# LiliMeng/network_interpretation_imagenet

Hardware: AMD Instinct MI355X
Metric: masked-forward-passes/sec (224x224, resnet101) (higher is better)
Workload: dtype f16x3 (split-fp16 MFMA, fp32 accumulate); stem conv in fp32 by superposition over superpixels; 1 GPU; resnet101, 512 masks/image x 128 images per GPU (BASELINE configs[2]; x1 GPUs); images_per_gpu=128, masks_per_image=512, forward_batch=2340, num_cus=256, entry=MaskedForwardEngine.score_packed, stem=table, lib_stamp=cd5194694597393f7e4ba467b20fff02ebc9e9c5ea24d07d825e02e5c1091293, lib_stamp_matches_tree=True, product_library=True, parallelism=mask-batch shard x1 + one all_gather of scores

## Files before the change

### network_interpretation_imagenet_amd/csrc/mpx_api.hip

```cpp
#include "../../include/mpx.h"
#include "mpx_kernels.h"
#include "mpx_conv3p.h"
#include "mpx_conv3pp.h"
#include "mpx_conv256.h"
#include "mpx_conv256p.h"
#include "mpx_convx.h"
#include "mpx_convw.h"
#include "mpx_btail.h"
#include "mpx_stemtab.h"
#include "mpx_dw.h"
#include "mpx_fire.h"
#include "mpx_pool3c.h"
#include "mpx_shuffle.h"
#include "mpx_mbconv.h"
#include "mpx_gconv.h"
#include "mpx_gconvw.h"
#include "mpx_cnext.h"
#include "mpx_attn.h"

#include <algorithm>
#include <cmath>
#include <cstdarg>
#include <initializer_list>
#include <new>
// ... 141 lines not shown
    int side, bf, hp, a_pitch, b_pitch, b_offset;
};

struct ClipPool {
    int hin, stride, pad, pitch;
};

struct ProfRec {
    hipEvent_t t0, t1;
    int kind;
    int conv;
    int sub;
};

}

struct mpx_engine {
    int arch = 0, max_batch = 0, device = 0;
    int num_cus = 256;
    int img = MPX_IMG, in_ch = 3, ncls = MPX_NUM_CLASSES, logit_pitch = MPX_NUM_CLASSES;
    bool small = false;
    bool vgg = false;
    bool alexnet = false;
    bool densenet = false;
    std::vector<NormLayer> norms;
    bool mobilenet = false;
    std::vector<DwLayer> dws;
    bool squeezenet = false;
    bool googlenet = false;
    std::vector<ClipPool> pools3c;
    bool shufflenet = false;
    std::vector<ShuffleOp> shuffles;
    bool efficientnet = false;
    std::vector<SeLayer> ses;
    float* se_gate = nullptr;
    int se_pitch_max = 0;
    bool convnext = false;
    std::vector<LnLayer> lnorms;
    bool regnet = false;
    bool vit = false;
    int vit_T = 0, vit_D = 0;
    std::vector<AttnLayer> attns;
    float* cls_token = nullptr;
    float* pos_emb = nullptr;
    bool tokens_loaded = false;
    size_t act_elems_buf[4] = {0, 0, 0, 0};
    int n_act_bufs = kActBufs;
    size_t act_elems_per_image = 0;
    float* k0_scratch = nullptr;
    bool bottleneck = false;
    int feat = 0;
    std::vector<ConvLayer> convs;
    std::vector<Op> ops;
    std::vector<Op> ops_bt;
    std::vector<TailBlock> tails;
    int ops_bt_x = 0;
    bool fuse_bt = true;
    std::vector<Op> ops_pt;
    std::vector<Op> ops_pt0;
    std::vector<PointTail> ptails;
    int ops_pt_x = 0, ops_pt0_x = 0;
    bool fuse_pt = true;
    char* arena = nullptr;
    size_t arena_bytes = 0;
    char* tab_arena = nullptr;
    size_t tab_arena_bytes = 0;
    half_t* in_hi = nullptr;
    half_t* in_lo = nullptr;
    half_t* act_hi[kActBufs] = {};
    half_t* act_lo[kActBufs] = {};
    half_t* pool_hi = nullptr;
    half_t* pool_lo = nullptr;
    float* logits = nullptr;
    float* seg_scratch = nullptr;
    half_t* stem_hi = nullptr;
    half_t* stem_lo = nullptr;
    float* stem_w32 = nullptr;
    float* stem_s32 = nullptr;
    float* stem_t32 = nullptr;
    int* tab_cnt = nullptr;
    int* tab_off = nullptr;
    int* tab_lab = nullptr;
    int* tab_heavy = nullptr;
    float* tab_vec = nullptr;
    unsigned* tab_bits = nullptr;
    size_t tab_sizes[4] = {0, 0, 0, 0};
    int tab_S = -1;
    bool stem_w_loaded = false;
    std::vector<uint8_t> slot_src;
    std::string err;
    bool in_forward = false;
    unsigned last_kernels = 0;
    bool fuse_ds = true;
    bool fuse_pool = true;
    bool prof_on = false;
    std::vector<ProfRec> prof_pool;
    int prof_used = 0;
    hipStream_t prof_stream = nullptr;
#ifdef MPX_DIAG
    unsigned long long* stamps = nullptr;
#endif
};

namespace {

int fail(mpx_engine* h, int code, const char* fmt, ...) {
    if (h) {
        char buf[512];
        va_list ap;
        va_start(ap, fmt);
        vsnprintf(buf, sizeof buf, fmt, ap);
        va_end(ap);
        h->err = buf;
    }
    return code;
}

#define MPX_HIP(h, call)                                                                         \
    do {                                                                                         \
        hipError_t e_ = (call);                                                                  \
        if (e_ != hipSuccess)                                                                    \
            return fail((h), (int)e_, "%s failed: %s (%s:%d)", #call, hipGetErrorString(e_),     \
                        __FILE__, __LINE__);                                                     \
    } while (0)

#define MPX_SET_DEVICE(h)                                   \
    do {                                                    \
        if (!(h)->in_forward) MPX_HIP((h), hipSetDevice((h)->device)); \
    } while (0)

size_t round_up(size_t v, size_t a) { return (v + a - 1) / a * a; }

void set_name(char* dst, const std::string& s) {
    std::snprintf(dst, 48, "%s", s.c_str());
}

int default_tile(const mpx_conv_desc& d);
bool patch_eligible(const mpx_conv_desc& d);

constexpr int kGconvTile = 16;
constexpr int kGconvwTile = 18;

int build_topology_small(mpx_engine* h);
int build_topology_vgg(mpx_engine* h);
int build_topology_alexnet(mpx_engine* h);
int build_topology_densenet(mpx_engine* h);
int build_topology_mobilenet(mpx_engine* h);
int build_topology_squeezenet(mpx_engine* h);
int build_topology_googlenet(mpx_engine* h);
int build_topology_shufflenet(mpx_engine* h);
int build_topology_efficientnet(mpx_engine* h);
int build_topology_convnext(mpx_engine* h);
int build_topology_vit(mpx_engine* h);
int build_topology_regnet(mpx_engine* h);

int build_topology(mpx_engine* h) {
    if (h->arch == MPX_ARCH_MNIST_NET || (h->arch > MPX_ARCH_CIFAR_RESNET && h->arch < MPX_ARCH_CIFAR_RESNET + 1000))
        return build_topology_small(h);
    if (h->arch > MPX_ARCH_VGG && h->arch < MPX_ARCH_VGG_BN + 100) return build_topology_vgg(h);
    if (h->arch >= MPX_ARCH_ALEXNET && h->arch < MPX_ARCH_ALEXNET + 100) return build_topology_alexnet(h);
    if (h->arch >= MPX_ARCH_DENSENET && h->arch < MPX_ARCH_DENSENET + 1000) return build_topology_densenet(h);
    if (h->arch >= MPX_ARCH_MOBILENET && h->arch < MPX_ARCH_MOBILENET + 1000) return build_topology_mobilenet(h);
    if (h->arch >= MPX_ARCH_SQUEEZENET && h->arch < MPX_ARCH_SQUEEZENET + 1000) return build_topology_squeezenet(h);
    if (h->arch >= MPX_ARCH_GOOGLENET && h->arch < MPX_ARCH_GOOGLENET + 1000) return build_topology_googlenet(h);
    if (h->arch >= MPX_ARCH_SHUFFLENET && h->arch < MPX_ARCH_SHUFFLENET + 1000) return build_topology_shufflenet(h);
    if (h->arch >= MPX_ARCH_EFFICIENTNET && h->arch < MPX_ARCH_EFFICIENTNET + 1000) return build_topology_efficientnet(h);
// ... 2448 lines not shown
    if (bias) *bias = h->lnorms[k].beta;
    if (eps) *eps = h->lnorms[k].eps;
    return 0;
}

int mpx_num_norms(const mpx_engine* h) { return h ? (int)h->norms.size() : MPX_E_ARG; }

int mpx_norm_info(const mpx_engine* h, int k, mpx_norm_desc* out) {
    if (!h || !out || k < 0 || k >= (int)h->norms.size()) return MPX_E_ARG;
    *out = h->norms[k].d;
    return 0;
}

int mpx_load_norm(mpx_engine* h, int k, const float* gamma, const float* beta, const float* mean, const float* var, float eps) {
    if (!h) return MPX_E_ARG;
    if (k < 0 || k >= (int)h->norms.size()) return fail(h, MPX_E_ARG, "load_norm: bad norm index %d (this engine has %d)", k, (int)h->norms.size());
    NormLayer& nl = h->norms[k];
    if (!gamma || !beta || !mean || !var) return fail(h, MPX_E_ARG, "load_norm: BatchNorm tensors missing for %s", nl.d.name);
    const int n = nl.d.channels;
    std::vector<float> sc(n), sh(n);
    for (int c = 0; c < n; ++c) {
        const double s = (double)gamma[c] / std::sqrt((double)var[c] + (double)eps);
        sc[c] = (float)s;
        sh[c] = (float)((double)beta[c] - (double)mean[c] * s);
    }
    MPX_SET_DEVICE(h);
    MPX_HIP(h, hipMemcpy(nl.scale, sc.data(), (size_t)n * 4, hipMemcpyHostToDevice));
    MPX_HIP(h, hipMemcpy(nl.shift, sh.data(), (size_t)n * 4, hipMemcpyHostToDevice));
    nl.loaded = true;
    return 0;
}

int mpx_norm_params(const mpx_engine* h, int k, const float** scale, const float** shift) {
    if (!h || !scale || !shift || k < 0 || k >= (int)h->norms.size()) return MPX_E_ARG;
    *scale = h->norms[k].scale;
    *shift = h->norms[k].shift;
    return 0;
}

int mpx_mask_apply_normalize(mpx_engine* h, const uint8_t* img_u8_hwc, const float* img_f32_chw, const int32_t* seg,
                             const uint8_t* onoff, int M, int S, const float mean[3], const float std[3], int slot0,
                             float* out_f32_nchw, void* stream) {
    if (!h) return MPX_E_ARG;
    if (h->small) return fail(h, MPX_E_STATE, "mask_apply_normalize: this engine runs one of the small networks; use mpx_mask_apply_minmax");
    if ((img_u8_hwc == nullptr) == (img_f32_chw == nullptr))
        return fail(h, MPX_E_ARG, "mask_apply_normalize: exactly one of img_u8_hwc / img_f32_chw must be given");
    if (!seg || !onoff || M <= 0 || S <= 0) return fail(h, MPX_E_ARG, "mask_apply_normalize: null input or empty M/S");
    if (img_u8_hwc && (!mean || !std)) return fail(h, MPX_E_ARG, "mask_apply_normalize: mean/std required for u8 input");
    if (slot0 < 0 || slot0 + M > h->max_batch) return fail(h, MPX_E_STATE, "mask_apply_normalize: slots [%d,%d) exceed max_batch %d", slot0, slot0 + M, h->max_batch);
    const size_t lds = round_up((size_t)K0_MT * S, 16);
    if (lds > 64 * 1024) return fail(h, MPX_E_ARG, "mask_apply_normalize: S=%d too large (max %d)", S, 64 * 1024 / K0_MT);
    MaskParams p;
    std::memset(&p, 0, sizeof p);
    p.img_u8 = img_u8_hwc; p.img_f32 = img_f32_chw; p.seg = seg; p.onoff = onoff;
    p.out_hi = h->in_hi; p.out_lo = h->in_lo; p.out_f32 = out_f32_nchw;
    for (int c = 0; c < 3; ++c) {
        p.mean[c] = mean ? mean[c] : 0.f;
        p.std[c] = std ? std[c] : 1.f;
    }
    p.M = M; p.S = S; p.slot0 = slot0;
    p.size = MPX_IMG; p.pad_size = MPX_IMG_PAD; p.border = 3;
    MPX_SET_DEVICE(h);
    hipStream_t st = as_stream(stream);
    ProfScope ps(h, st, 1, -1);
    dim3 grid((MPX_IMG * MPX_IMG + 255) / 256, (M + K0_MT - 1) / K0_MT);
    hipLaunchKernelGGL(mask_apply_normalize_kernel, grid, dim3(256), lds, st, p);
    MPX_HIP(h, hipGetLastError());
    std::fill(h->slot_src.begin() + slot0, h->slot_src.begin() + slot0 + M, (uint8_t)1);
    return 0;
}

int mpx_stem_table_build(mpx_engine* h, const uint8_t* img_u8_hwc, const float* img_f32_chw, const int32_t* seg, int S,
                         const float mean[3], const float std[3], void* stream) {
    if (!h) return MPX_E_ARG;
    if (h->densenet) return fail(h, MPX_E_STATE, "stem_table_build: a DenseNet engine keeps no stem table; it stages through mpx_mask_apply_normalize");
    if (!h->stem_w32) return fail(h, MPX_E_STATE, "stem_table_build: this architecture has no 7x7 stem with a max pool%s", h->vgg || h->alexnet || h->mobilenet || h->squeezenet || h->googlenet || h->shufflenet || h->efficientnet || h->convnext || h->vit || h->regnet ? " (VGG, AlexNet, MobileNetV2, SqueezeNet, GoogLeNet, ShuffleNetV2, EfficientNet-B0, ConvNeXt, ViT and RegNetX stage through mpx_mask_apply_normalize)" : "");
    if ((img_u8_hwc == nullptr) == (img_f32_chw == nullptr))
        return fail(h, MPX_E_ARG, "stem_table_build: exactly one of img_u8_hwc / img_f32_chw must be given");
    if (!seg || S <= 0 || S > 4096) return fail(h, MPX_E_ARG, "stem_table_build: null label map or S outside [1, 4096]");
    if (img_u8_hwc && (!mean || !std)) return fail(h, MPX_E_ARG, "stem_table_build: mean/std required for u8 input");
    if (!h->stem_w_loaded) return fail(h, MPX_E_STATE, "stem_table_build: layer 0 (%s) has no weights", h->convs[0].d.name);
    MPX_SET_DEVICE(h);
    if (!h->tab_arena) {
        const size_t total = 3 * h->tab_sizes[0] + h->tab_sizes[1] + h->tab_sizes[2] + h->tab_sizes[3];
        MPX_HIP(h, hipMalloc((void**)&h->tab_arena, total));
        h->tab_arena_bytes = total;
        char* cur = h->tab_arena;
        auto take = [&](size_t n) { char* r = cur; cur += n; return r; };
        h->tab_cnt = (int*)take(h->tab_sizes[0]);
        h->tab_off = (int*)take(h->tab_sizes[0]);
        h->tab_heavy = (int*)take(h->tab_sizes[0]);
        h->tab_lab = (int*)take(h->tab_sizes[1]);
        h->tab_vec = (float*)take(h->tab_sizes[2]);
        h->tab_bits = (unsigned*)take(h->tab_sizes[3]);
    }
    StemTabParams p;
    std::memset(&p, 0, sizeof p);
    p.img_u8 = img_u8_hwc; p.img_f32 = img_f32_chw; p.seg = seg; p.S = S;
    for (int c = 0; c < 3; ++c) {
        p.mean[c] = mean ? mean[c] : 0.f;
        p.std[c] = std ? std[c] : 1.f;
    }
    p.w = h->stem_w32; p.cnt = h->tab_cnt; p.off = h->tab_off; p.lab = h->tab_lab; p.vec = h->tab_vec;
    MPX_SET_DEVICE(h);
    hipStream_t st = as_stream(stream);
    ProfScope ps(h, st, 1, -1);
    hipLaunchKernelGGL(stemtab_count_kernel, dim3(ST_NPIX / 4), dim3(256), 0, st, p);
    MPX_HIP(h, hipGetLastError());
    hipLaunchKernelGGL(stemtab_scan_kernel, dim3(1), dim3(1024), 0, st, (const int*)h->tab_cnt, h->tab_off);
    MPX_HIP(h, hipGetLastError());
    hipLaunchKernelGGL(stemtab_fill_kernel, dim3(ST_NPIX / 4), dim3(256), 0, st, p);
    MPX_HIP(h, hipGetLastError());
    hipLaunchKernelGGL(stemtab_heavy_kernel, dim3(1), dim3(1024), 0, st, (const int*)h->tab_off, h->tab_heavy, h->tab_heavy + ST_POOLED * ST_POOLED);
    MPX_HIP(h, hipGetLastError());
    h->tab_S = S;
    return 0;
}

int mpx_stem_table_apply(mpx_engine* h, const uint8_t* onoff, int M, int S, int slot0, void* stream) {
    if (!h) return MPX_E_ARG;
    if (h->densenet) return fail(h, MPX_E_STATE, "stem_table_apply: a DenseNet engine keeps no stem table; it stages through mpx_mask_apply_normalize");
    if (!h->stem_w32) return fail(h, MPX_E_STATE, "stem_table_apply: this architecture has no 7x7 stem with a max pool");
    if (!onoff || M <= 0) return fail(h, MPX_E_ARG, "stem_table_apply: null mask rows or empty M");
    if (h->tab_S < 0) return fail(h, MPX_E_STATE, "stem_table_apply: no table in place (mpx_stem_table_build first; loading layer 0 again discards it)");
    if (S != h->tab_S) return fail(h, MPX_E_ARG, "stem_table_apply: S=%d, the table was built with S=%d", S, h->tab_S);
    if (slot0 < 0 || slot0 + M > h->max_batch) return fail(h, MPX_E_STATE, "stem_table_apply: slots [%d,%d) exceed max_batch %d", slot0, slot0 + M, h->max_batch);
    const int nmb = (M + 31) / 32;
    MPX_SET_DEVICE(h);
    hipStream_t st = as_stream(stream);
    {
        ProfScope ps(h, st, 1, -1);
        hipLaunchKernelGGL(onoff_bitplanes_kernel, dim3((S * nmb + 255) / 256), dim3(256), 0, st, onoff, M, S, nmb, h->tab_bits);
        MPX_HIP(h, hipGetLastError());
    }
    StemApplyParams p;
    std::memset(&p, 0, sizeof p);
    p.off = h->tab_off; p.lab = h->tab_lab; p.vec = h->tab_vec; p.bits = h->tab_bits; p.s = h->stem_s32; p.t = h->stem_t32;
    p.out_hi = h->stem_hi; p.out_lo = h->stem_lo; p.nmb = nmb; p.M = M; p.slot0 = slot0;
    p.heavy_list = h->tab_heavy; p.heavy_count = h->tab_heavy + ST_POOLED * ST_POOLED;
    {
        ProfScope ps(h, st, OP_CONV, 0);
        hipLaunchKernelGGL(stem_apply_heavy_kernel, dim3(h->num_cus, nmb), dim3(256), 0, st, p);
        MPX_HIP(h, hipGetLastError());
        hipLaunchKernelGGL(stem_apply_kernel, dim3(ST_POOLED * ST_POOLED / 4, nmb), dim3(256), 0, st, p);
        MPX_HIP(h, hipGetLastError());
    }
    std::fill(h->slot_src.begin() + slot0, h->slot_src.begin() + slot0 + M, (uint8_t)2);
    return 0;
}

int mpx_mask_apply_minmax(mpx_engine* h, const float* img_f32_chw, const int32_t* seg, const uint8_t* removed, int M, int S,
                          int slot0, float* out_f32_nchw, void* stream) {
    if (!h) return MPX_E_ARG;
    if (!h->small) return fail(h, MPX_E_STATE, "mask_apply_minmax: only the small networks (MNIST net, CIFAR ResNet) use this mask convention");
    if (!img_f32_chw || !seg || !removed || M <= 0 || S <= 0 || S > 4096) return fail(h, MPX_E_ARG, "mask_apply_minmax: null input, empty M/S or S > 4096");
    if (slot0 < 0 || slot0 + M > h->max_batch) return fail(h, MPX_E_STATE, "mask_apply_minmax: slots [%d,%d) exceed max_batch %d", slot0, slot0 + M, h->max_batch);
    MPX_SET_DEVICE(h);
    hipStream_t st = as_stream(stream);
    ProfScope ps(h, st, 1, -1);
    const int hw = h->img * h->img;
    float* stats = h->k0_scratch;
    float* mask_max = h->k0_scratch + 2 + 4096;
    hipLaunchKernelGGL(smallnet_image_stats_kernel, dim3(1), dim3(256), 0, st, img_f32_chw, seg, h->in_ch, hw, S, stats);
    MPX_HIP(h, hipGetLastError());
    hipLaunchKernelGGL(smallnet_mask_max_kernel, dim3((M + 255) / 256), dim3(256), 0, st, removed, M, S, (const float*)stats, mask_max);
    MPX_HIP(h, hipGetLastError());
    SmallMaskParams p;
    std::memset(&p, 0, sizeof p);
    p.img = img_f32_chw; p.seg = seg; p.removed = removed; p.stats = stats; p.mask_max = mask_max;
    p.out_hi = h->in_hi; p.out_lo = h->in_lo; p.out_f32 = out_f32_nchw;
    p.C = h->in_ch; p.hw = hw; p.M = M; p.S = S; p.slot0 = slot0;
    hipLaunchKernelGGL(smallnet_mask_apply_kernel, dim3((hw + 255) / 256, M), dim3(256), 0, st, p);
    MPX_HIP(h, hipGetLastError());
    return 0;
}

int mpx_avgpool2_pad(mpx_engine* h, const void* in_hi, const void* in_lo, void* out_hi, void* out_lo, int B, int hin,
                     int cin_p, int cout_p, void* stream) {
    if (!h) return MPX_E_ARG;
    if (!in_hi || !in_lo || !out_hi || !out_lo || B <= 0 || hin <= 0 || (hin & 1) || cin_p <= 0 || (cin_p & 7) || cout_p < cin_p || (cout_p & 7))
        return fail(h, MPX_E_ARG, "avgpool2_pad: bad arguments (hin even, channel counts multiples of 8, cout_p >= cin_p)");
    if (((uintptr_t)in_hi | (uintptr_t)in_lo | (uintptr_t)out_hi | (uintptr_t)out_lo) & 15)
        return fail(h, MPX_E_ARG, "avgpool2_pad: the planes must be 16-byte aligned");
    MPX_SET_DEVICE(h);
    hipStream_t st = as_stream(stream);
    ProfScope ps(h, st, 2, -1);
    const size_t total = (size_t)B * (hin / 2) * (hin / 2) * (cout_p / 8);
    const unsigned grid = (unsigned)std::min<size_t>((total + 255) / 256, 256 * 64);
    hipLaunchKernelGGL(avgpool2_pad_kernel, dim3(grid), dim3(256), 0, st, (const half_t*)in_hi, (const half_t*)in_lo,
                       (half_t*)out_hi, (half_t*)out_lo, B, hin, cin_p, cout_p);
    MPX_HIP(h, hipGetLastError());
    return 0;
}

int mpx_geometry(const mpx_engine* h, int* image_size, int* in_channels, int* num_classes, int* logit_pitch) {
    if (!h) return MPX_E_ARG;
    if (image_size) *image_size = h->img;
    if (in_channels) *in_channels = h->in_ch;
    if (num_classes) *num_classes = h->ncls;
    if (logit_pitch) *logit_pitch = h->logit_pitch;
    return 0;
}

int mpx_conv_bn_act(mpx_engine* h, int i, const void* in_hi, const void* in_lo, const void* res_hi, const void* res_lo,
                    void* out_hi, void* out_lo, float* out_f32, int B, void* stream) {
    if (!h) return MPX_E_ARG;
    if (i < 0 || i >= (int)h->convs.size() || B <= 0) return fail(h, MPX_E_ARG, "conv_bn_act: bad layer index or batch");
    const ConvLayer& L = h->convs[i];
    if (L.is_stem) {
        if (in_hi || in_lo) return fail(h, MPX_E_ARG, "conv_bn_act: layer 0 reads the engine input staging; pass NULL inputs");
        if (B > h->max_batch) return fail(h, MPX_E_STATE, "conv_bn_act: B > max_batch");
    } else if (h->small && i == 0 && !in_hi && !in_lo) {
        in_hi = h->in_hi;
        in_lo = h->in_lo;
        if (B > h->max_batch) return fail(h, MPX_E_STATE, "conv_bn_act: B > max_batch");
    } else if (!in_hi || !in_lo) {
        return fail(h, MPX_E_ARG, "conv_bn_act: null input planes");
    }
    if ((res_hi == nullptr) != (res_lo == nullptr)) return fail(h, MPX_E_ARG, "conv_bn_act: residual planes must come in pairs");
    if (L.is_fc ? (out_f32 == nullptr) : (out_f32 != nullptr || !out_hi || !out_lo))
        return fail(h, MPX_E_ARG, "conv_bn_act: fc writes out_f32, every other layer writes out_hi/out_lo");
    MPX_SET_DEVICE(h);
    return launch_conv(h, i, (const half_t*)in_hi, (const half_t*)in_lo, (const half_t*)res_hi, (const half_t*)res_lo,
                       (half_t*)out_hi, (half_t*)out_lo, out_f32, B, as_stream(stream));
}

// ... 1104 lines not shown
```

### network_interpretation_imagenet_amd/csrc/mpx_stemtab.h

```cpp
#pragma once
#include "mpx_conv.h"

namespace mpx {

constexpr int ST_IN = 224, ST_CONV = 112, ST_POOLED = 56, ST_TAPS = 49, ST_C = 64;
constexpr int ST_NPIX = ST_CONV * ST_CONV;
constexpr int ST_MAX_ENTRIES = ST_NPIX * ST_TAPS;

struct StemTabParams {
    const uint8_t* img_u8;
    const float* img_f32;
    const int32_t* seg;
    float mean[3], std[3];
    int S;
    const float* w;
    int* cnt;
    int* off;
    int* lab;
    float* vec;
};

__device__ __forceinline__ int st_tap_label(const StemTabParams& p, int oy, int ox, int t, int* pix_out) {
    const int ky = t / 7, kx = t - ky * 7;
    const int iy = 2 * oy - 3 + ky, ix = 2 * ox - 3 + kx;
// ... 35 lines not shown
    for (int d = 1; d < 1024; d <<= 1) {
        const int v = t >= d ? s[t - d] : 0;
        __syncthreads();
        s[t] += v;
        __syncthreads();
    }
    int run = s[t] - sum;
    for (int i = 0; i < PER; ++i)
        if (base + i < ST_NPIX) {
            off[base + i] = run;
            run += cnt[base + i];
        }
    if (t == 1023) off[ST_NPIX] = s[1023];
}

__global__ __launch_bounds__(256) void stemtab_fill_kernel(const StemTabParams p) {
    __shared__ int s_lab[4][64];
    __shared__ float s_x[4][3][64];
    const int lane = threadIdx.x & 63, wave = threadIdx.x >> 6;
    const int q = blockIdx.x * 4 + wave;
    const int oy = q / ST_CONV, ox = q - oy * ST_CONV;
    int pix = 0;
    const int l = lane < ST_TAPS ? st_tap_label(p, oy, ox, lane, &pix) : -1;
    float x[3] = {0.f, 0.f, 0.f};
    if (l >= 0) {
        if (p.img_u8) {
#pragma unroll
            for (int c = 0; c < 3; ++c) {
                const float t = __fdiv_rn((float)p.img_u8[(size_t)pix * 3 + c], 255.0f);
                x[c] = __fdiv_rn(__fsub_rn(t, p.mean[c]), p.std[c]);
            }
        } else {
#pragma unroll
            for (int c = 0; c < 3; ++c) x[c] = p.img_f32[(size_t)c * ST_IN * ST_IN + pix];
        }
    }
    s_lab[wave][lane] = l;
#pragma unroll
    for (int c = 0; c < 3; ++c) s_x[wave][c][lane] = x[c];
    __syncthreads();
    unsigned long long firsts = st_first_occurrences(s_lab[wave], lane, l);
    int e = p.off[q];
    const float* w = p.w + lane;
    while (firsts) {
        const int t0 = __ffsll((long long)firsts) - 1;
        firsts &= firsts - 1;
        const int u = s_lab[wave][t0];
        float acc = 0.f;
        for (int t = t0; t < ST_TAPS; ++t) {
            if (s_lab[wave][t] != u) continue;
#pragma unroll
            for (int c = 0; c < 3; ++c) acc = fmaf(w[(t * 3 + c) * ST_C], s_x[wave][c][t], acc);
        }
        p.vec[(size_t)e * ST_C + lane] = acc;
        if (lane == 0) p.lab[e] = u;
        ++e;
    }
}

__global__ __launch_bounds__(256) void onoff_bitplanes_kernel(const uint8_t* __restrict__ onoff, int M, int S, int nmb,
                                                              unsigned* __restrict__ bits) {
    const int i = blockIdx.x * 256 + threadIdx.x;
    if (i >= S * nmb) return;
    const int mb = i / S, s = i - mb * S;
    unsigned w = 0;
    for (int j = 0; j < 32; ++j) {
        const int m = mb * 32 + j;
        if (m < M && onoff[(size_t)m * S + s]) w |= 1u << j;
    }
    bits[(size_t)s * nmb + mb] = w;
}

struct StemApplyParams {
    const int* __restrict__ off;
    const int* __restrict__ lab;
    const float* __restrict__ vec;
    const unsigned* __restrict__ bits;
    const float* __restrict__ s;
    const float* __restrict__ t;
    half_t* __restrict__ out_hi;
    half_t* __restrict__ out_lo;
    const int* __restrict__ heavy_list;
    const int* __restrict__ heavy_count;
    int nmb, M, slot0;
};

__device__ __forceinline__ void stem_store4_packed(const StemApplyParams& p, unsigned (*s_out)[4][4][ST_C], int m, int mcount, int wave, int lane,
                                                   unsigned packed, size_t out0_row) {
    s_out[(m >> 2) & 1][m & 3][wave][lane] = packed;
    if ((m & 3) != 3 && m != mcount - 1) return;
    __syncthreads();
    const int ms = (m & ~3) + wave;
    if (ms < mcount) {
        typedef unsigned u4 __attribute__((ext_vector_type(4)));
        typedef unsigned u2 __attribute__((ext_vector_type(2)));
        const u4 q = *(const u4*)&s_out[(m >> 2) & 1][ms & 3][lane >> 4][(lane & 15) * 4];
        u2 vh, vl;
        vh[0] = (q[0] & 0xffffu) | (q[1] << 16);
        vh[1] = (q[2] & 0xffffu) | (q[3] << 16);
        vl[0] = (q[0] >> 16) | (q[1] & 0xffff0000u);
        vl[1] = (q[2] >> 16) | (q[3] & 0xffff0000u);
        const size_t o = out0_row + (size_t)ms * ST_POOLED * ST_POOLED * ST_C + (size_t)(lane >> 4) * ST_C + (lane & 15) * 4;
        __builtin_nontemporal_store(vh, (u2*)(p.out_hi + o));
        __builtin_nontemporal_store(vl, (u2*)(p.out_lo + o));
    }
}

__device__ __forceinline__ unsigned stem_split_packed(float best) {
    half_t hi, lo;
    split_f32(best, hi, lo);
    const unsigned lob = __builtin_bit_cast(unsigned short, lo);
    return (unsigned)__builtin_bit_cast(unsigned short, hi) | ((lob == 0x8000u ? 0u : lob) << 16);
}

__device__ __forceinline__ void stem_store4(const StemApplyParams& p, unsigned (*s_out)[4][4][ST_C], int m, int mcount, int wave, int lane,
                                            float best, size_t out0_row) {
    stem_store4_packed(p, s_out, m, mcount, wave, lane, stem_split_packed(best), out0_row);
}

struct StemRows {
    int a0, l0, a1, l1, a2, l2;
    int o00, o01, o02, o10, o11, o12, o20, o21, o22;
};

__device__ __forceinline__ void stem_entry(const StemRows& w, int i, int& g, bool& start) {
    if (i < w.l0) {
        g = w.a0 + i;
        start = g == w.o00 || g == w.o01 || g == w.o02;
    } else if (i < w.l0 + w.l1) {
        g = w.a1 + (i - w.l0);
        start = g == w.o10 || g == w.o11 || g == w.o12;
    } else {
        g = w.a2 + (i - w.l0 - w.l1);
        start = g == w.o20 || g == w.o21 || g == w.o22;
    }
}

constexpr int SA_CH = 32, SA_MG = 8;

__device__ __forceinline__ void stem_load_chunk(const StemApplyParams& p, const StemRows& w, int cb, int n_e, int lane, int mb,
                                                float (&R)[SA_CH], unsigned& starts, unsigned& kbv) {
    const int cnt = min(SA_CH, n_e - cb);
    starts = 0;
#pragma unroll
    for (int i = 0; i < SA_CH; ++i) {
        int g = 0;
        bool st = false;
        stem_entry(w, cb + i, g, st);
        const bool ok = i < cnt;
        R[i] = ok ? p.vec[(size_t)g * ST_C + lane] : 0.f;
        if (ok && st && cb + i > 0) starts |= 1u << i;
    }
    kbv = 0;
    if (lane < cnt) {
        int g = 0;
        bool st = false;
        stem_entry(w, cb + lane, g, st);
        kbv = p.bits[(size_t)p.lab[g] * p.nmb + mb];
    }
}

constexpr int SA_KF_PITCH = 56;

template <int KPP, bool BORDER>
__device__ __forceinline__ void stem_apply_fast(const StemApplyParams& p, unsigned (*s_out)[4][4][ST_C], float (*s_kf)[SA_KF_PITCH], int wave,
                                                int lane, int mcount, size_t out0_row, const int (&o)[9], const int (&len)[9],
                                                const bool (&qok)[9], float sc, float sh, int mb) {
    constexpr int NS = 9 * KPP, NS4 = (NS + 3) / 4 * 4;
    float R[NS4];
#pragma unroll
    for (int q = 0; q < 9; ++q)
#pragma unroll
        for (int k = 0; k < KPP; ++k) {
            const bool ok = k < len[q];
            const int g = o[q] + k;
            R[q * KPP + k] = ok ? p.vec[(size_t)g * ST_C + lane] : 0.f;
            const unsigned kb = ok ? p.bits[(size_t)p.lab[g] * p.nmb + mb] : 0u;
            if (lane < 32) s_kf[lane][q * KPP + k] = (kb >> lane & 1u) ? 1.0f : 0.0f;
        }
#pragma unroll
    for (int i = NS; i < NS4; ++i) {
        R[i] = 0.f;
        if (lane < 32) s_kf[lane][i] = 0.f;
    }
    __builtin_amdgcn_fence(__ATOMIC_RELEASE, "wavefront");
    __builtin_amdgcn_wave_barrier();
    __builtin_amdgcn_fence(__ATOMIC_ACQUIRE, "wavefront");
    for (int m = 0; m < mcount; ++m) {
        f4 kf[NS4 / 4];
#pragma unroll
        for (int i = 0; i < NS4 / 4; ++i) kf[i] = *(const f4*)&s_kf[m][4 * i];
        float best = -INFINITY;
#pragma unroll
        for (int q = 0; q < 9; ++q) {
            float v = 0.f;
#pragma unroll
            for (int k = 0; k < KPP; ++k)
                v = fmaf(kf[(q * KPP + k) / 4][(q * KPP + k) % 4], R[q * KPP + k], v);
            const float y = fmaxf(fmaf(v, sc, sh), 0.f);
            best = fmaxf(best, BORDER ? (qok[q] ? y : -INFINITY) : y);
        }
        stem_store4(p, s_out, m, mcount, wave, lane, best, out0_row);
    }
}

struct StemPixel {
    StemRows w;
    int n_e, n_empty, kmax;
    int o9[9], len9[9];
    bool qok[9];
    bool interior;
};

__device__ __forceinline__ void stem_pixel(const StemApplyParams& p, int py, int px, StemPixel& g) {
    const int cx0 = max(2 * px - 1, 0);
    const int ncol = 2 * px + 1 - cx0 + 1;
    StemRows& w = g.w;
    g.n_empty = 0;
    {
        const int cy0 = 2 * py - 1, cy1 = 2 * py, cy2 = 2 * py + 1;
        const bool ok0 = cy0 >= 0;
        const int q0 = (ok0 ? cy0 : 0) * ST_CONV + cx0, q1 = cy1 * ST_CONV + cx0, q2 = cy2 * ST_CONV + cx0;
        const int e00 = p.off[q0], e01 = p.off[q0 + 1], e02 = p.off[q0 + 2], e03 = p.off[q0 + ncol];
        const int e10 = p.off[q1], e11 = p.off[q1 + 1], e12 = p.off[q1 + 2], e13 = p.off[q1 + ncol];
        const int e20 = p.off[q2], e21 = p.off[q2 + 1], e22 = p.off[q2 + 2], e23 = p.off[q2 + ncol];
        w.a0 = e00; w.l0 = ok0 ? e03 - e00 : 0; w.o00 = e00; w.o01 = e01; w.o02 = e02;
        w.a1 = e10; w.l1 = e13 - e10; w.o10 = e10; w.o11 = e11; w.o12 = e12;
        w.a2 = e20; w.l2 = e23 - e20; w.o20 = e20; w.o21 = e21; w.o22 = e22;
        if (ok0) g.n_empty += (e01 == e00) + (e02 == e01) + (ncol == 3 && e03 == e02);
        g.n_empty += (e11 == e10) + (e12 == e11) + (ncol == 3 && e13 == e12);
        g.n_empty += (e21 == e20) + (e22 == e21) + (ncol == 3 && e23 == e22);
    }
    g.n_e = w.l0 + w.l1 + w.l2;
    const bool col0_ok = px > 0, row0_ok = py > 0;
    const int e0[4] = {w.o00, w.o01, w.o02, w.a0 + w.l0}, e1[4] = {w.o10, w.o11, w.o12, w.a1 + w.l1}, e2[4] = {w.o20, w.o21, w.o22, w.a2 + w.l2};
    g.kmax = 0;
#pragma unroll
    for (int c = 0; c < 3; ++c) {
        const bool cok = col0_ok || c > 0;
        const int j = cok ? (col0_ok ? c : c - 1) : 0;
        g.qok[c] = cok && row0_ok;
        g.qok[3 + c] = cok;
        g.qok[6 + c] = cok;
        g.o9[c] = e0[j];
        g.o9[3 + c] = e1[j];
        g.o9[6 + c] = e2[j];
        g.len9[c] = g.qok[c] ? e0[j + 1] - e0[j] : 0;
        g.len9[3 + c] = cok ? e1[j + 1] - e1[j] : 0;
        g.len9[6 + c] = cok ? e2[j + 1] - e2[j] : 0;
    }
#pragma unroll
    for (int q = 0; q < 9; ++q) g.kmax = max(g.kmax, g.len9[q]);
    g.interior = col0_ok && row0_ok;
}

__device__ __forceinline__ bool stem_heavy(const StemPixel& g) { return !(g.kmax <= 6 && (g.kmax <= 4 || g.interior)); }

__global__ __launch_bounds__(1024) void stemtab_heavy_kernel(const int* __restrict__ off, int* __restrict__ heavy_list, int* __restrict__ heavy_count) {
    __shared__ int s_n;
    if (threadIdx.x == 0) s_n = 0;
    __syncthreads();
    StemApplyParams p;
    p.off = off;
    for (int P = threadIdx.x; P < ST_POOLED * ST_POOLED; P += 1024) {
        StemPixel g;
        stem_pixel(p, P / ST_POOLED, P % ST_POOLED, g);
        if (stem_heavy(g)) heavy_list[atomicAdd(&s_n, 1)] = P;
    }
    __syncthreads();
    if (threadIdx.x == 0) *heavy_count = s_n;
}

__global__ __launch_bounds__(256) void stem_apply_heavy_kernel(const StemApplyParams p) {
    __shared__ __attribute__((aligned(16))) float s_ks[4][SA_MG * SA_CH];
    const int lane = threadIdx.x & 63;
    const int wave = __builtin_amdgcn_readfirstlane(threadIdx.x >> 6);
    const int mb = blockIdx.y;
    const int mw0 = wave * SA_MG;
    const int mcount = min(SA_MG, p.M - (mb * 32 + mw0));
    if (mcount <= 0) return;
    const float sc = p.s[lane], sh = p.t[lane];
    const float y_empty = fmaxf(sh, 0.f);
    const int n_heavy = *p.heavy_count;
    float* ks = s_ks[wave];
  for (int hi_ = blockIdx.x; hi_ < n_heavy; hi_ += gridDim.x) {
    const int P = p.heavy_list[hi_];
    const int py = P / ST_POOLED, px = P - py * ST_POOLED;
    StemPixel g;
    stem_pixel(p, py, px, g);
    float v[SA_MG], best[SA_MG];
#pragma unroll
    for (int k = 0; k < SA_MG; ++k) {
        v[k] = 0.f;
        best[k] = g.n_empty > 0 ? y_empty : -INFINITY;
    }
    for (int cb = 0; cb < g.n_e; cb += SA_CH) {
        const int cnt = min(SA_CH, g.n_e - cb);
        float R[SA_CH];
        unsigned starts = 0, kbv = 0;
        stem_load_chunk(p, g.w, cb, g.n_e, lane, mb, R, starts, kbv);
        __builtin_amdgcn_wave_barrier();
        if (lane < SA_CH) {
#pragma unroll
            for (int k = 0; k < SA_MG; ++k) ks[k * SA_CH + lane] = (kbv >> (mw0 + k) & 1u) ? 1.0f : 0.0f;
        }
        __builtin_amdgcn_fence(__ATOMIC_RELEASE, "wavefront");
        __builtin_amdgcn_wave_barrier();
        __builtin_amdgcn_fence(__ATOMIC_ACQUIRE, "wavefront");
#pragma unroll
        for (int k = 0; k < SA_MG; ++k) {
#pragma unroll
            for (int i4 = 0; i4 < SA_CH / 4; ++i4) {
                const f4 kf = *(const f4*)&ks[k * SA_CH + 4 * i4];
#pragma unroll
                for (int ii = 0; ii < 4; ++ii) {
                    const int i = 4 * i4 + ii;
                    if (i < cnt) {
                        if (starts >> i & 1) {
                            asm volatile("" ::: "memory");
                            best[k] = fmaxf(best[k], fmaxf(fmaf(v[k], sc, sh), 0.f));
                            v[k] = 0.f;
                        }
                        v[k] = fmaf(kf[ii], R[i], v[k]);
                    }
                }
            }
        }
    }
    const size_t out0 = (((size_t)(p.slot0 + mb * 32 + mw0) * ST_POOLED + py) * ST_POOLED + px) * ST_C + lane;
#pragma unroll
    for (int k = 0; k < SA_MG; ++k) {
        if (k < mcount) {
            const float b = g.n_e > 0 ? fmaxf(best[k], fmaxf(fmaf(v[k], sc, sh), 0.f)) : best[k];
            const unsigned packed = stem_split_packed(b);
            const size_t o = out0 + (size_t)k * ST_POOLED * ST_POOLED * ST_C;
            p.out_hi[o] = __builtin_bit_cast(half_t, (unsigned short)(packed & 0xffffu));
            p.out_lo[o] = __builtin_bit_cast(half_t, (unsigned short)(packed >> 16));
        }
    }
    __builtin_amdgcn_wave_barrier();
  }
}

__global__ __launch_bounds__(256) void stem_apply_kernel(const StemApplyParams p) {
    __shared__ __attribute__((aligned(16))) unsigned s_out[2][4][4][ST_C];
    __shared__ __attribute__((aligned(16))) float s_kf[4][32][SA_KF_PITCH];
    const int lane = threadIdx.x & 63;
    const int wave = __builtin_amdgcn_readfirstlane(threadIdx.x >> 6);
    const int P = blockIdx.x * 4 + wave;
    const int mb = blockIdx.y;
    const int m0 = mb * 32;
    const int mcount = min(32, p.M - m0);
    const int py = P / ST_POOLED, px = P - py * ST_POOLED;
    StemPixel g;
    stem_pixel(p, py, px, g);
    const float sc = p.s[lane], sh = p.t[lane];
    const size_t out0_row = (((size_t)(p.slot0 + m0) * ST_POOLED + py) * ST_POOLED + (px - wave)) * ST_C;
    if (stem_heavy(g)) {
        const size_t o0 = out0_row + (size_t)wave * ST_C + lane;
        for (int m = 0; m < mcount; ++m) {
            const size_t o = o0 + (size_t)m * ST_POOLED * ST_POOLED * ST_C;
            const unsigned packed = (unsigned)__builtin_bit_cast(unsigned short, p.out_hi[o]) | ((unsigned)__builtin_bit_cast(unsigned short, p.out_lo[o]) << 16);
            stem_store4_packed(p, s_out, m, mcount, wave, lane, packed, out0_row);
        }
    } else if (g.interior) {
        if (g.kmax <= 1) stem_apply_fast<1, false>(p, s_out, s_kf[wave], wave, lane, mcount, out0_row, g.o9, g.len9, g.qok, sc, sh, mb);
        else if (g.kmax <= 2) stem_apply_fast<2, false>(p, s_out, s_kf[wave], wave, lane, mcount, out0_row, g.o9, g.len9, g.qok, sc, sh, mb);
        else if (g.kmax <= 3) stem_apply_fast<3, false>(p, s_out, s_kf[wave], wave, lane, mcount, out0_row, g.o9, g.len9, g.qok, sc, sh, mb);
        else if (g.kmax <= 4) stem_apply_fast<4, false>(p, s_out, s_kf[wave], wave, lane, mcount, out0_row, g.o9, g.len9, g.qok, sc, sh, mb);
        else stem_apply_fast<6, false>(p, s_out, s_kf[wave], wave, lane, mcount, out0_row, g.o9, g.len9, g.qok, sc, sh, mb);
    } else {
        if (g.kmax <= 2) stem_apply_fast<2, true>(p, s_out, s_kf[wave], wave, lane, mcount, out0_row, g.o9, g.len9, g.qok, sc, sh, mb);
        else stem_apply_fast<4, true>(p, s_out, s_kf[wave], wave, lane, mcount, out0_row, g.o9, g.len9, g.qok, sc, sh, mb);
    }
}

}
```

Measured before the change: 24320 masked-forward-passes/s.

## Precompute stem outputs per superpixel on/off pattern and look them up per mask

At table-build time, pooled stem pixels covered by at most four distinct superpixel labels are marked, and those labels are recorded. At apply time such pixel groups evaluate the stem once for each of the 16 on/off combinations into LDS. Each mask's output is then a table lookup indexed by its keep bits, written with nontemporal stores, so per-mask FMA work is replaced by copies. It adds a build kernel, a per-block pattern check and extra table memory, and the per-block work now spans several mask blocks, which lowers the number of active blocks.

```diff
diff --git a/network_interpretation_imagenet_amd/csrc/mpx_api.hip b/network_interpretation_imagenet_amd/csrc/mpx_api.hip
--- a/network_interpretation_imagenet_amd/csrc/mpx_api.hip
+++ b/network_interpretation_imagenet_amd/csrc/mpx_api.hip
@@ -247,6 +247,7 @@
     int* tab_off = nullptr;
     int* tab_lab = nullptr;
     int* tab_heavy = nullptr;
+    int* tab_pat = nullptr;
     float* tab_vec = nullptr;
     unsigned* tab_bits = nullptr;
     size_t tab_sizes[4] = {0, 0, 0, 0};
@@ -2861,7 +2862,7 @@
     if (!h->stem_w_loaded) return fail(h, MPX_E_STATE, "stem_table_build: layer 0 (%s) has no weights", h->convs[0].d.name);
     MPX_SET_DEVICE(h);
     if (!h->tab_arena) {
-        const size_t total = 3 * h->tab_sizes[0] + h->tab_sizes[1] + h->tab_sizes[2] + h->tab_sizes[3];
+        const size_t total = 4 * h->tab_sizes[0] + h->tab_sizes[1] + h->tab_sizes[2] + h->tab_sizes[3];
         MPX_HIP(h, hipMalloc((void**)&h->tab_arena, total));
         h->tab_arena_bytes = total;
         char* cur = h->tab_arena;
@@ -2869,6 +2870,8 @@
         h->tab_cnt = (int*)take(h->tab_sizes[0]);
         h->tab_off = (int*)take(h->tab_sizes[0]);
         h->tab_heavy = (int*)take(h->tab_sizes[0]);
+        static_assert(ST_POOLED * ST_POOLED * SP_NP <= ST_NPIX + 1, "tab_pat is one int vector of the table");
+        h->tab_pat = (int*)take(h->tab_sizes[0]);
         h->tab_lab = (int*)take(h->tab_sizes[1]);
         h->tab_vec = (float*)take(h->tab_sizes[2]);
         h->tab_bits = (unsigned*)take(h->tab_sizes[3]);
@@ -2892,6 +2895,9 @@
     MPX_HIP(h, hipGetLastError());
     hipLaunchKernelGGL(stemtab_heavy_kernel, dim3(1), dim3(1024), 0, st, (const int*)h->tab_off, h->tab_heavy, h->tab_heavy + ST_POOLED * ST_POOLED);
     MPX_HIP(h, hipGetLastError());
+    hipLaunchKernelGGL(stemtab_pattern_kernel, dim3((ST_POOLED * ST_POOLED + 255) / 256), dim3(256), 0, st, (const int*)h->tab_off, (const int*)h->tab_lab,
+                       h->tab_pat);
+    MPX_HIP(h, hipGetLastError());
     h->tab_S = S;
     return 0;
 }
@@ -2917,10 +2923,12 @@
     p.off = h->tab_off; p.lab = h->tab_lab; p.vec = h->tab_vec; p.bits = h->tab_bits; p.s = h->stem_s32; p.t = h->stem_t32;
     p.out_hi = h->stem_hi; p.out_lo = h->stem_lo; p.nmb = nmb; p.M = M; p.slot0 = slot0;
     p.heavy_list = h->tab_heavy; p.heavy_count = h->tab_heavy + ST_POOLED * ST_POOLED;
+    p.pat_lab = h->tab_pat;
     {
         ProfScope ps(h, st, OP_CONV, 0);
         hipLaunchKernelGGL(stem_apply_heavy_kernel, dim3(h->num_cus, nmb), dim3(256), 0, st, p);
         MPX_HIP(h, hipGetLastError());
+        p.patterns = M >= SP_MIN_M;
         hipLaunchKernelGGL(stem_apply_kernel, dim3(ST_POOLED * ST_POOLED / 4, nmb), dim3(256), 0, st, p);
         MPX_HIP(h, hipGetLastError());
     }
diff --git a/network_interpretation_imagenet_amd/csrc/mpx_stemtab.h b/network_interpretation_imagenet_amd/csrc/mpx_stemtab.h
--- a/network_interpretation_imagenet_amd/csrc/mpx_stemtab.h
+++ b/network_interpretation_imagenet_amd/csrc/mpx_stemtab.h
@@ -141,7 +141,9 @@
     half_t* __restrict__ out_lo;
     const int* __restrict__ heavy_list;
     const int* __restrict__ heavy_count;
+    const int* __restrict__ pat_lab;
     int nmb, M, slot0;
+    int patterns;
 };
 
 __device__ __forceinline__ void stem_store4_packed(const StemApplyParams& p, unsigned (*s_out)[4][4][ST_C], int m, int mcount, int wave, int lane,
@@ -221,46 +223,58 @@
 
 constexpr int SA_KF_PITCH = 56;
 
+__device__ __forceinline__ void stem_wave_sync() {
+    __builtin_amdgcn_fence(__ATOMIC_RELEASE, "wavefront");
+    __builtin_amdgcn_wave_barrier();
+    __builtin_amdgcn_fence(__ATOMIC_ACQUIRE, "wavefront");
+}
+
+template <int KPP, bool BORDER, int NR, int PITCH, class KeepWord, class Sink>
+__device__ __forceinline__ void stem_eval_static(const StemApplyParams& p, float (*s_kf)[PITCH], int lane, int mcount, const int (&o)[9],
+                                                 const int (&len)[9], const bool (&qok)[9], float sc, float sh, KeepWord keep_word, Sink sink) {
+    constexpr int NS = 9 * KPP, NS4 = (NS + 3) / 4 * 4;
+    float R[NS4];
+#pragma unroll
+    for (int q = 0; q < 9; ++q)
+#pragma unroll
+        for (int k = 0; k < KPP; ++k) {
+            const bool ok = k < len[q];
+            const int g = o[q] + k;
+            R[q * KPP + k] = ok ? p.vec[(size_t)g * ST_C + lane] : 0.f;
+            const unsigned kb = ok ? keep_word(g) : 0u;
+            if (lane < NR) s_kf[lane][q * KPP + k] = (kb >> lane & 1u) ? 1.0f : 0.0f;
+        }
+#pragma unroll
+    for (int i = NS; i < NS4; ++i) {
+        R[i] = 0.f;
+        if (lane < NR) s_kf[lane][i] = 0.f;
+    }
+    stem_wave_sync();
+    for (int m = 0; m < mcount; ++m) {
+        f4 kf[NS4 / 4];
+#pragma unroll
+        for (int i = 0; i < NS4 / 4; ++i) kf[i] = *(const f4*)&s_kf[m][4 * i];
+        float best = -INFINITY;
+#pragma unroll
+        for (int q = 0; q < 9; ++q) {
+            float v = 0.f;
+#pragma unroll
+            for (int k = 0; k < KPP; ++k)
+                v = fmaf(kf[(q * KPP + k) / 4][(q * KPP + k) % 4], R[q * KPP + k], v);
+            const float y = fmaxf(fmaf(v, sc, sh), 0.f);
+            best = fmaxf(best, BORDER ? (qok[q] ? y : -INFINITY) : y);
+        }
+        sink(m, best);
+    }
+}
+
 template <int KPP, bool BORDER>
 __device__ __forceinline__ void stem_apply_fast(const StemApplyParams& p, unsigned (*s_out)[4][4][ST_C], float (*s_kf)[SA_KF_PITCH], int wave,
                                                 int lane, int mcount, size_t out0_row, const int (&o)[9], const int (&len)[9],
                                                 const bool (&qok)[9], float sc, float sh, int mb) {
-    constexpr int NS = 9 * KPP, NS4 = (NS + 3) / 4 * 4;
-    float R[NS4];
-#pragma unroll
-    for (int q = 0; q < 9; ++q)
-#pragma unroll
-        for (int k = 0; k < KPP; ++k) {
-            const bool ok = k < len[q];
-            const int g = o[q] + k;
-            R[q * KPP + k] = ok ? p.vec[(size_t)g * ST_C + lane] : 0.f;
-            const unsigned kb = ok ? p.bits[(size_t)p.lab[g] * p.nmb + mb] : 0u;
-            if (lane < 32) s_kf[lane][q * KPP + k] = (kb >> lane & 1u) ? 1.0f : 0.0f;
-        }
-#pragma unroll
-    for (int i = NS; i < NS4; ++i) {
-        R[i] = 0.f;
-        if (lane < 32) s_kf[lane][i] = 0.f;
-    }
-    __builtin_amdgcn_fence(__ATOMIC_RELEASE, "wavefront");
-    __builtin_amdgcn_wave_barrier();
-    __builtin_amdgcn_fence(__ATOMIC_ACQUIRE, "wavefront");
-    for (int m = 0; m < mcount; ++m) {
-        f4 kf[NS4 / 4];
-#pragma unroll
-        for (int i = 0; i < NS4 / 4; ++i) kf[i] = *(const f4*)&s_kf[m][4 * i];
-        float best = -INFINITY;
-#pragma unroll
-        for (int q = 0; q < 9; ++q) {
-            float v = 0.f;
-#pragma unroll
-            for (int k = 0; k < KPP; ++k)
-                v = fmaf(kf[(q * KPP + k) / 4][(q * KPP + k) % 4], R[q * KPP + k], v);
-            const float y = fmaxf(fmaf(v, sc, sh), 0.f);
-            best = fmaxf(best, BORDER ? (qok[q] ? y : -INFINITY) : y);
-        }
-        stem_store4(p, s_out, m, mcount, wave, lane, best, out0_row);
-    }
+    stem_eval_static<KPP, BORDER, 32, SA_KF_PITCH>(
+        p, s_kf, lane, mcount, o, len, qok, sc, sh, [&](int g) { return p.bits[(size_t)p.lab[g] * p.nmb + mb]; },
+        [&](int m, float best) { stem_store4(p, s_out, m, mcount, wave, lane, best, out0_row); });
 }
 
 struct StemPixel {
@@ -315,6 +329,18 @@
 
 __device__ __forceinline__ bool stem_heavy(const StemPixel& g) { return !(g.kmax <= 6 && (g.kmax <= 4 || g.interior)); }
 
+constexpr int SP_NP = 4;
+constexpr int SP_PROWS = 1 << SP_NP;
+constexpr int SP_PW = 4;
+constexpr int SP_DIRECT = -2;
+#ifndef MPX_STEMPAT_MBW
+#define MPX_STEMPAT_MBW 4
+#endif
+#ifndef MPX_STEMPAT_MIN_M
+#define MPX_STEMPAT_MIN_M 48
+#endif
+constexpr int SP_MBW = MPX_STEMPAT_MBW, SP_MIN_M = MPX_STEMPAT_MIN_M;
+
 __global__ __launch_bounds__(1024) void stemtab_heavy_kernel(const int* __restrict__ off, int* __restrict__ heavy_list, int* __restrict__ heavy_count) {
     __shared__ int s_n;
     if (threadIdx.x == 0) s_n = 0;
@@ -328,6 +354,43 @@
     }
     __syncthreads();
     if (threadIdx.x == 0) *heavy_count = s_n;
+}
+
+__global__ __launch_bounds__(256) void stemtab_pattern_kernel(const int* __restrict__ off, const int* __restrict__ lab, int* __restrict__ pat_lab) {
+    static_assert(SP_NP == 4, "the label registers below");
+    const int P = blockIdx.x * 256 + threadIdx.x;
+    if (P >= ST_POOLED * ST_POOLED) return;
+    StemApplyParams p;
+    p.off = off;
+    StemPixel g;
+    stem_pixel(p, P / ST_POOLED, P % ST_POOLED, g);
+    int l[9 * SP_NP];
+#pragma unroll
+    for (int q = 0; q < 9; ++q)
+#pragma unroll
+        for (int k = 0; k < SP_NP; ++k) l[q * SP_NP + k] = k < g.len9[q] ? lab[g.o9[q] + k] : -1;
+    int l0 = -1, l1 = -1, l2 = -1, l3 = -1, n = 0;
+#pragma unroll
+    for (int i = 0; i < 9 * SP_NP; ++i) {
+        const int v = l[i];
+        if (v < 0 || v == l0 || v == l1 || v == l2 || v == l3) continue;
+        if (n == 0) l0 = v;
+        else if (n == 1) l1 = v;
+        else if (n == 2) l2 = v;
+        else if (n == 3) l3 = v;
+        ++n;
+    }
+    const bool direct = stem_heavy(g) || g.kmax > SP_NP || n > SP_NP;
+    pat_lab[P * SP_NP + 0] = direct ? SP_DIRECT : l0;
+    pat_lab[P * SP_NP + 1] = direct ? -1 : l1;
+    pat_lab[P * SP_NP + 2] = direct ? -1 : l2;
+    pat_lab[P * SP_NP + 3] = direct ? -1 : l3;
+}
+
+__device__ __forceinline__ bool stem_pattern_group(const StemApplyParams& p, int P0) {
+    static_assert(SP_PW == 4, "the four loads below");
+    return p.pat_lab[P0 * SP_NP] != SP_DIRECT && p.pat_lab[(P0 + 1) * SP_NP] != SP_DIRECT && p.pat_lab[(P0 + 2) * SP_NP] != SP_DIRECT &&
+           p.pat_lab[(P0 + 3) * SP_NP] != SP_DIRECT;
 }
 
 __global__ __launch_bounds__(256) void stem_apply_heavy_kernel(const StemApplyParams p) {
@@ -401,9 +464,80 @@
   }
 }
 
+template <int NR, int PITCH, class KeepWord, class Sink>
+__device__ __forceinline__ void stem_eval_pixel(const StemApplyParams& p, const StemPixel& g, float (*s_kf)[PITCH], int lane, int mcount, float sc,
+                                                float sh, KeepWord keep_word, Sink sink) {
+    if (g.interior) {
+        if (g.kmax <= 1) stem_eval_static<1, false, NR, PITCH>(p, s_kf, lane, mcount, g.o9, g.len9, g.qok, sc, sh, keep_word, sink);
+        else if (g.kmax <= 2) stem_eval_static<2, false, NR, PITCH>(p, s_kf, lane, mcount, g.o9, g.len9, g.qok, sc, sh, keep_word, sink);
+        else if (g.kmax <= 3) stem_eval_static<3, false, NR, PITCH>(p, s_kf, lane, mcount, g.o9, g.len9, g.qok, sc, sh, keep_word, sink);
+        else if (g.kmax <= 4) stem_eval_static<4, false, NR, PITCH>(p, s_kf, lane, mcount, g.o9, g.len9, g.qok, sc, sh, keep_word, sink);
+        else stem_eval_static<6, false, NR, PITCH>(p, s_kf, lane, mcount, g.o9, g.len9, g.qok, sc, sh, keep_word, sink);
+    } else {
+        if (g.kmax <= 2) stem_eval_static<2, true, NR, PITCH>(p, s_kf, lane, mcount, g.o9, g.len9, g.qok, sc, sh, keep_word, sink);
+        else stem_eval_static<4, true, NR, PITCH>(p, s_kf, lane, mcount, g.o9, g.len9, g.qok, sc, sh, keep_word, sink);
+    }
+}
+
+__device__ __forceinline__ void stem_apply_patterns(const StemApplyParams& p, unsigned (*s_row)[SP_PROWS][ST_C], int mbg) {
+    static_assert(SP_NP == 4 && SP_PW == 4 && ST_POOLED % SP_PW == 0, "lane layout and label registers below");
+    static_assert(SA_KF_PITCH <= ST_C, "a pattern's keep factors fit its row");
+    typedef unsigned u4 __attribute__((ext_vector_type(4)));
+    const int lane = threadIdx.x & 63;
+    const int wave = __builtin_amdgcn_readfirstlane(threadIdx.x >> 6);
+    const int P0 = blockIdx.x * SP_PW, P = P0 + wave;
+    const int mb0 = mbg * SP_MBW, mb1 = min(mb0 + SP_MBW, p.nmb);
+    const float sc = p.s[lane], sh = p.t[lane];
+    {
+        const int l0 = p.pat_lab[P * SP_NP], l1 = p.pat_lab[P * SP_NP + 1], l2 = p.pat_lab[P * SP_NP + 2], l3 = p.pat_lab[P * SP_NP + 3];
+        const int n = (l0 >= 0) + (l1 >= 0) + (l2 >= 0) + (l3 >= 0);
+        float(*kf)[ST_C] = (float(*)[ST_C]) & s_row[wave][0][0];
+        unsigned short* tab = (unsigned short*)&s_row[wave][0][0];
+        StemPixel g;
+        stem_pixel(p, P / ST_POOLED, P % ST_POOLED, g);
+        stem_eval_pixel<SP_PROWS>(p, g, kf, lane, 1 << n, sc, sh,
+                                  [&](int e) {
+                                      const int l = p.lab[e];
+                                      return l == l0 ? 0xAAAAu : l == l1 ? 0xCCCCu : l == l2 ? 0xF0F0u : 0xFF00u;
+                                  },
+                                  [&](int m, float best) {
+                                      const unsigned pk = stem_split_packed(best);
+                                      tab[m * (2 * ST_C) + lane] = (unsigned short)(pk & 0xffffu);
+                                      tab[m * (2 * ST_C) + ST_C + lane] = (unsigned short)(pk >> 16);
+                                  });
+    }
+    __syncthreads();
+    const int msel = lane >> 5, ps = (lane >> 3) & 3, j8 = lane & 7;
+    const char* tabp = (const char*)&s_row[ps][0][0] + j8 * 16;
+    const size_t plane = (size_t)ST_POOLED * ST_POOLED * ST_C;
+    const size_t o0 = ((size_t)p.slot0 * ST_POOLED * ST_POOLED + P0 + ps) * ST_C + j8 * 8;
+    const int* pl = p.pat_lab + (P0 + ps) * SP_NP;
+    const int L0 = pl[0], L1 = pl[1], L2 = pl[2], L3 = pl[3];
+    for (int mb = mb0; mb < mb1; ++mb) {
+        const unsigned kw0 = L0 >= 0 ? p.bits[(size_t)L0 * p.nmb + mb] : 0u, kw1 = L1 >= 0 ? p.bits[(size_t)L1 * p.nmb + mb] : 0u;
+        const unsigned kw2 = L2 >= 0 ? p.bits[(size_t)L2 * p.nmb + mb] : 0u, kw3 = L3 >= 0 ? p.bits[(size_t)L3 * p.nmb + mb] : 0u;
+#pragma unroll
+        for (int it = 0; it < 4; ++it) {
+            const unsigned ml = (wave + 4 * it) * 2 + msel;
+            const unsigned row = (kw0 >> ml & 1u) | (kw1 >> ml & 1u) << 1 | (kw2 >> ml & 1u) << 2 | (kw3 >> ml & 1u) << 3;
+            const u4 vh = *(const u4*)(tabp + row * (ST_C * 4)), vl = *(const u4*)(tabp + row * (ST_C * 4) + ST_C * 2);
+            const int m = mb * 32 + (int)ml;
+            if (m < p.M) {
+                __builtin_nontemporal_store(vh, (u4*)(p.out_hi + o0 + m * plane));
+                __builtin_nontemporal_store(vl, (u4*)(p.out_lo + o0 + m * plane));
+            }
+        }
+    }
+}
+
 __global__ __launch_bounds__(256) void stem_apply_kernel(const StemApplyParams p) {
     __shared__ __attribute__((aligned(16))) unsigned s_out[2][4][4][ST_C];
     __shared__ __attribute__((aligned(16))) float s_kf[4][32][SA_KF_PITCH];
+    static_assert(sizeof(s_kf) >= sizeof(unsigned) * SP_PW * SP_PROWS * ST_C, "the pattern tables fit the keep factors' LDS");
+    if (p.patterns && stem_pattern_group(p, blockIdx.x * 4)) {
+        if (blockIdx.y * SP_MBW < p.nmb) stem_apply_patterns(p, (unsigned(*)[SP_PROWS][ST_C]) & s_kf[0][0][0], blockIdx.y);
+        return;
+    }
     const int lane = threadIdx.x & 63;
     const int wave = __builtin_amdgcn_readfirstlane(threadIdx.x >> 6);
     const int P = blockIdx.x * 4 + wave;
```

Result: no change. 24500 masked-forward-passes/s (median of 6 runs) (+0.7%).
